# bruno-maruszczak/lap-time-optimization

Measured on AMD Instinct MI355X. Metric: MPC solves/sec (N=40, nx=8 [7 + progress s], nu=2), higher is better.
Workload: dtype f64

## Files before the change

lap-time-optimization_amd/csrc/aux_kernels.h:

```cpp
#pragma once
#include "linearise.h"

namespace ltompc {

template <bool PI = false, bool TS = false>
__device__ __forceinline__ void d_init_slot(const Consts& K, const Work& W, const int k, const int b, const int cold) {
  const int N = W.N;
  double x0[8];
#pragma unroll
  for (int i = 0; i < 8; i++) x0[i] = W.x0[(size_t)i * W.Bp + b];
  if (k == 0) {
#pragma unroll
    for (int i = 0; i < 8; i++) PL(W.X, i, 0, N + 1) = x0[i];
  }
  if (cold) {
#pragma unroll
    for (int i = 0; i < 8; i++) {
      PL(W.X, i, k + 1, N + 1) = x0[i], PL(W.C, i, k, N) = x0[i];
      PL(W.L1, i, k, N) = 0.0, PL(W.L2, i, k, N) = 0.0;
    }
    PL(W.U, 0, k, N) = 0.0, PL(W.U, 1, k, N) = 0.0;
  }
  const int prev = W.si[(size_t)SI_PREV * W.Bp + b];
  const bool resto_ok = K.o.resto_rho > 0.0 && !(K.o.soft_rho > 0.0);
// ... 52 lines not shown
  int b = tid % W.Bp, k = tid / W.Bp;
  if (k >= W.N || b >= W.B) return;
  d_init_slot(K, W, k, b, cold);
}
__global__ void k_init_pi(const Consts* __restrict__ Kp, const WorkPI* __restrict__ Wp, int cold) {
  const Consts& K = *Kp;
  const Work& W = *Wp;
  int tid = blockIdx.x * blockDim.x + threadIdx.x;
  int b = tid % W.Bp, k = tid / W.Bp;
  if (k >= W.N || b >= W.B) return;
  d_init_slot<true>(K, W, k, b, cold);
}
__global__ void k_init_ts(const Consts* __restrict__ Kp, const WorkTS* __restrict__ Wp, int cold) {
  const Consts& K = *Kp;
  const Work& W = *Wp;
  int tid = blockIdx.x * blockDim.x + threadIdx.x;
  int b = tid % W.Bp, k = tid / W.Bp;
  if (k >= W.N || b >= W.B) return;
  d_init_slot<true, true>(K, W, k, b, cold);
}

__global__ void k_shift(Work W, int pass) {
  int tid = blockIdx.x * blockDim.x + threadIdx.x;
  int b = tid % W.Bp, k = tid / W.Bp;
  const int N = W.N;
  if (k > N || b >= W.B) return;
  if (pass == 0) {
    const int kx = k + 1 <= N ? k + 1 : N, ks = k + 1 <= N - 1 ? k + 1 : N - 1;
#pragma unroll
    for (int i = 0; i < 8; i++) PL(W.dX, i, k, N + 1) = PL(W.X, i, kx, N + 1);
    if (k < N) {
#pragma unroll
      for (int i = 0; i < 8; i++) {
        PL(W.dC, i, k, N) = PL(W.C, i, ks, N);
        PL(W.nL1, i, k, N) = PL(W.L1, i, ks, N), PL(W.nL2, i, k, N) = PL(W.L2, i, ks, N);
      }
      PL(W.dU, 0, k, N) = PL(W.U, 0, ks, N), PL(W.dU, 1, k, N) = PL(W.U, 1, ks, N);
    }
  } else {
#pragma unroll
    for (int i = 0; i < 8; i++) PL(W.X, i, k, N + 1) = PL(W.dX, i, k, N + 1);
    if (k < N) {
#pragma unroll
      for (int i = 0; i < 8; i++) {
        PL(W.C, i, k, N) = PL(W.dC, i, k, N);
        PL(W.L1, i, k, N) = PL(W.nL1, i, k, N), PL(W.L2, i, k, N) = PL(W.nL2, i, k, N);
      }
      PL(W.U, 0, k, N) = PL(W.dU, 0, k, N), PL(W.U, 1, k, N) = PL(W.dU, 1, k, N);
    }
  }
}


__global__ void k_act_identity(int* act, int* nact, int B) {
  int b = blockIdx.x * blockDim.x + threadIdx.x;
  if (b < B) act[b] = b;
  if (b == 0) nact[0] = B;
}
__global__ void __launch_bounds__(1024) k_compact(const int* __restrict__ src, const int* __restrict__ nsrc_p,
                                                   const int* __restrict__ done, int* __restrict__ dst, int* __restrict__ ndst) {
  __shared__ int cnt[1024];
  const int t = threadIdx.x, nsrc = nsrc_p[0];
  const int chunk = (nsrc + 1023) / 1024, lo = t * chunk, hi = min(nsrc, lo + chunk);
  int c = 0;
  for (int j = lo; j < hi; j++) c += done[src[j]] ? 0 : 1;
  cnt[t] = c;
  __syncthreads();
  for (int off = 1; off < 1024; off <<= 1) {
    int v = t >= off ? cnt[t - off] : 0;
    __syncthreads();
    cnt[t] += v;
    __syncthreads();
  }
  int pos = cnt[t] - c;
  for (int j = lo; j < hi; j++) {
    int b = src[j];
    if (!done[b]) dst[pos++] = b;
  }
  if (t == 1023) ndst[0] = cnt[1023];
}

__global__ void __launch_bounds__(1024) k_pack_perm(const int* __restrict__ nslots_p, const int* __restrict__ done, int* __restrict__ perm,
                                                     int* __restrict__ act, int* __restrict__ nact) {
  __shared__ int cnt[1024];
  const int t = threadIdx.x, n = nslots_p[0];
  const int chunk = (n + 1023) / 1024, lo = min(n, t * chunk), hi = min(n, lo + chunk);
  int c = 0;
  for (int j = lo; j < hi; j++) c += done[j] ? 0 : 1;
  cnt[t] = c;
  __syncthreads();
  for (int off = 1; off < 1024; off <<= 1) {
    int v = t >= off ? cnt[t - off] : 0;
    __syncthreads();
    cnt[t] += v;
    __syncthreads();
  }
  const int n_act = cnt[1023];
  int pa = cnt[t] - c, pd = n_act + lo - pa;
  for (int j = lo; j < hi; j++) {
    if (!done[j]) act[pa] = pa, perm[pa++] = j;
    else perm[pd++] = j;
  }
  if (t == 0) nact[0] = n_act;
}
__global__ void k_pack_inverse(const int* __restrict__ orig, int* __restrict__ inv, int B) {
  int j = blockIdx.x * blockDim.x + threadIdx.x;
// ... 247 lines not shown
```

lap-time-optimization_amd/csrc/linesearch.h:

```cpp
#pragma once
#include "layout.h"

namespace ltompc {

template <class BP, bool PIN, bool ELL, bool PI = false, bool TS = false>
__device__ __forceinline__ void d_linesearch(const Consts& K, const Work& W, const int k, const int b, const int l_begin,
                                             const int l_end) {
  const int N = W.N;
  const double hdt = K.o.t_step;
  if (W.si[(size_t)SI_DONE * W.Bp + b] || !W.si[(size_t)SI_STEP * W.Bp + b]) return;
  const double eps = W.st[(size_t)ST_EPS * W.Bp + b], rho = W.st[(size_t)ST_RHO * W.Bp + b];
  double a_pri = 1.0;
  for (int kk = 0; kk < N; kk += 20) {
    double v20[20];
#pragma unroll
    for (int q = 0; q < 20; q++) v20[q] = PL(W.SP, SP_apri, kk + q < N ? kk + q : N - 1, N);
#pragma unroll
    for (int q = 0; q < 20; q++) a_pri = fmin(a_pri, v20[q]);
  }
  double xk[8], xp[8], c[8], u[2], v[2], dxk[8], dxp[8], dc[8], du[2], dv[2];
#pragma unroll
  for (int i = 0; i < 8; i++) {
    xk[i] = k == 0 ? W.x0[(size_t)i * W.Bp + b] : PL(W.X, i, k, N + 1);
    dxk[i] = PL(W.dX, i, k, N + 1);
// ... 428 lines not shown
    u[0] = PL(W.U, 0, k, N), u[1] = PL(W.U, 1, k, N), du[0] = PL(W.dU, 0, k, N), du[1] = PL(W.dU, 1, k, N);
#pragma unroll
    for (int i = 0; i < 8; i++) {
      PL(W.X, i, k + 1, N + 1) = x[i] + alpha * dx[i];
      PL(W.C, i, k, N) = c[i] + alpha * dc[i];
      PL(W.L1, i, k, N) = l1[i] + alpha * (n1[i] - l1[i]);
      PL(W.L2, i, k, N) = l2[i] + alpha * (n2[i] - l2[i]);
    }
    PL(W.U, 0, k, N) = u[0] + alpha * du[0], PL(W.U, 1, k, N) = u[1] + alpha * du[1];
  }
  const int ni = K.bd.ni, nel = K.bd.nel, nact = (k + 1 <= N - 1) ? ni : ni - 3 - nel;
  for (int m0 = 0; m0 < nact; m0 += 8) {
    double t[8], dt[8], nu[8], dn[8];
#pragma unroll
    for (int q = 0; q < 8; q++) {
      const int m = m0 + q < nact ? m0 + q : nact - 1;
      t[q] = PL(W.T, m, k, N), dt[q] = PL(W.dT, m, k, N), nu[q] = PL(W.NU, m, k, N), dn[q] = PL(W.dNU, m, k, N);
    }
#pragma unroll
    for (int q = 0; q < 8; q++)
      if (m0 + q < nact) {
        const double tn = t[q] + alpha * dt[q];
        const double nn = nu[q] + a_dua * dn[q];
        const double lo = mu / (1e10 * tn), hi = 1e10 * mu / tn;
        PL(W.T, m0 + q, k, N) = tn, PL(W.NU, m0 + q, k, N) = nn < lo ? lo : (nn > hi ? hi : nn);
      }
  }
  if (W.st[(size_t)ST_RHO * W.Bp + b] > 0.0 && nact == ni) {
    double e[3], de[3];
#pragma unroll
    for (int q = 0; q < 3; q++) e[q] = PL(W.T, ni + q, k, N), de[q] = PL(W.dT, ni + q, k, N);
#pragma unroll
    for (int q = 0; q < 3; q++) PL(W.T, ni + q, k, N) = e[q] + alpha * de[q];
  }
  if (nel && nact == ni) {
    double e[2], de[2];
#pragma unroll
    for (int q = 0; q < 2; q++) e[q] = PL(W.T, ni + 3 + q, k, N), de[q] = PL(W.dT, ni + 3 + q, k, N);
#pragma unroll
    for (int q = 0; q < 2; q++) PL(W.T, ni + 3 + q, k, N) = e[q] + alpha * de[q];
  }
}

__global__ void __launch_bounds__(64) k_update(const Consts* __restrict__ Kp, const Work* __restrict__ Wp, Launch la) {
  const Consts& K = *Kp;
  const Work& W = *Wp;
  int tid = blockIdx.x * blockDim.x + threadIdx.x;
  if (tid == 0) W.ls_count[1] = W.ls_count[0], W.ls_count[0] = 0;
  int j = tid % la.n_pad, k = tid / la.n_pad;
  if (k >= W.N || j >= la.nact[0]) return;
  d_update(K, W, k, la.act[j]);
}


template <class BP, bool ELL>
__global__ void __launch_bounds__(320) k_step1(const Consts* __restrict__ Kp, const Work* __restrict__ Wp, Launch la) {
  const Consts& K = *Kp;
  const Work& W = *Wp;
  if ((int)blockIdx.x >= la.nact[0]) return;
  const int b = la.act[blockIdx.x];
  const int N = W.N, tid = threadIdx.x;
  const int* si = W.si;
  if (si[(size_t)SI_DONE * W.Bp + b] || !si[(size_t)SI_STEP * W.Bp + b]) return;
  const bool rprof = W.DBG != nullptr && blockIdx.x == 0 && tid == 0;
  long long rt0 = rprof ? clock64() : 0;
#define STOCK(q) if (rprof) { const long long t1 = clock64(); W.DBG[q] += (double)(t1 - rt0); rt0 = t1; }
  for (int idx = tid; idx < N * K.o.n_linesearch; idx += 320) d_linesearch<BP, false, ELL>(K, W, idx % N, b, 1 + idx / N, 1 + idx / N);
  STOCK(8);
  __syncthreads();
  STOCK(9);
  if (tid < 64 && (tid & 7) == 0) d_pick(K, W, b, tid >> 3, 1, false);
  __syncthreads();
  STOCK(10);
  for (int kk = tid; kk < N; kk += 320) d_update(K, W, kk, b);
  STOCK(11);
  if (rprof) W.DBG[12] += 1.0;
#undef STOCK
}
template <class BP>
__global__ void __launch_bounds__(320) k_step1_pi(const Consts* __restrict__ Kp, const WorkPI* __restrict__ Wp, Launch la) {
  const Consts& K = *Kp;
  const Work& W = *Wp;
  if ((int)blockIdx.x >= la.nact[0]) return;
  const int b = la.act[blockIdx.x];
  const int N = W.N, tid = threadIdx.x;
  const int* si = W.si;
  if (si[(size_t)SI_DONE * W.Bp + b] || !si[(size_t)SI_STEP * W.Bp + b]) return;
  const bool rprof = W.DBG != nullptr && blockIdx.x == 0 && tid == 0;
  long long rt0 = rprof ? clock64() : 0;
#define STOCK(q) if (rprof) { const long long t1 = clock64(); W.DBG[q] += (double)(t1 - rt0); rt0 = t1; }
  for (int idx = tid; idx < N * K.o.n_linesearch; idx += 320) d_linesearch<BP, false, false, true>(K, W, idx % N, b, 1 + idx / N, 1 + idx / N);
  STOCK(8);
  __syncthreads();
  STOCK(9);
  if (tid < 64 && (tid & 7) == 0) d_pick<true>(K, W, b, tid >> 3, 1, false);
  __syncthreads();
  STOCK(10);
  for (int kk = tid; kk < N; kk += 320) d_update(K, W, kk, b);
  STOCK(11);
  if (rprof) W.DBG[12] += 1.0;
#undef STOCK
}
template <class BP>
__global__ void __launch_bounds__(320) k_step1_ts(const Consts* __restrict__ Kp, const WorkTS* __restrict__ Wp, Launch la) {
  const Consts& K = *Kp;
  const Work& W = *Wp;
  if ((int)blockIdx.x >= la.nact[0]) return;
  const int b = la.act[blockIdx.x];
  const int N = W.N, tid = threadIdx.x;
  const int* si = W.si;
  if (si[(size_t)SI_DONE * W.Bp + b] || !si[(size_t)SI_STEP * W.Bp + b]) return;
  const bool rprof = W.DBG != nullptr && blockIdx.x == 0 && tid == 0;
  long long rt0 = rprof ? clock64() : 0;
#define STOCK(q) if (rprof) { const long long t1 = clock64(); W.DBG[q] += (double)(t1 - rt0); rt0 = t1; }
  for (int idx = tid; idx < N * K.o.n_linesearch; idx += 320) d_linesearch<BP, false, false, true, true>(K, W, idx % N, b, 1 + idx / N, 1 + idx / N);
  STOCK(8);
  __syncthreads();
  STOCK(9);
  if (tid < 64 && (tid & 7) == 0) d_pick<true, true>(K, W, b, tid >> 3, 1, false);
  __syncthreads();
  STOCK(10);
  for (int kk = tid; kk < N; kk += 320) d_update(K, W, kk, b);
  STOCK(11);
  if (rprof) W.DBG[12] += 1.0;
#undef STOCK
}



}
```

lap-time-optimization_amd/csrc/ltompc.hip:

```cpp
#include <hip/hip_runtime.h>

#include <algorithm>
#include <cmath>
#include <cstdio>
#include <cstdlib>
#include <cstring>
#include <string>
#include <type_traits>
#include <vector>

#include "kernels.h"

using namespace ltompc;

namespace {

thread_local std::string g_err;

int fail(const std::string& msg) {
  g_err = msg;
  return -1;
}
#define HIPCHECK(expr)                                                                         \
  do {                                                                                         \
    hipError_t e_ = (expr);                                                                    \
    if (e_ != hipSuccess) return fail(std::string(#expr) + ": " + hipGetErrorString(e_));      \
  } while (0)

constexpr int NKERN = 8;

}

enum class Sens { no_solve, solved, du0, traj };
enum class Psens { none, du0, traj };
struct DerivState {
  Sens sens = Sens::no_solve;
  Psens psens = Psens::none;
  bool fact = false;
  bool pv_valid = false;
  bool kept_uprev = false;
  bool loop_fresh = false;
  int loop_mode = 0;

  void discard() { sens = Sens::no_solve, psens = Psens::none, fact = pv_valid = kept_uprev = false; }
  void solved(const bool kept_u) { sens = Sens::solved, kept_uprev = kept_u, loop_fresh = loop_fresh || kept_u; }
  void moved() { fact = pv_valid = false; }
  void ticked() { loop_fresh = false; }

  Work Ws{}, *d_Ws = nullptr;
  WorkPI Wspi{}, *d_Wspi = nullptr;
  int *d_sens_inertia = nullptr, *d_sens_ok = nullptr;
  double *d_sens_du0 = nullptr, *d_sens_margin = nullptr, *d_sens_dX = nullptr, *d_sens_dU = nullptr;
  double *d_psens_uprev = nullptr, *d_psens_pv = nullptr, *d_psens_kf = nullptr, *d_psens_du0 = nullptr, *d_psens_dX = nullptr,
         *d_psens_dU = nullptr;
  double *d_adj_aj = nullptr, *d_adj_gp = nullptr, *d_adj_gth = nullptr, *d_adj_gX = nullptr, *d_adj_gU = nullptr;
  double *d_psn_planes = nullptr, *d_psn_rm = nullptr, *d_loop_Sx = nullptr, *d_loop_Du = nullptr;
  double *d_jvp_jv = nullptr, *d_jvp_dp = nullptr, *d_jvp_dth = nullptr, *d_jvp_tX = nullptr, *d_jvp_tU = nullptr;
  int *d_loop_ok = nullptr, *d_loop_ticks = nullptr;
  double *d_tab_tj = nullptr, *d_tab_sg = nullptr, *d_tab_gt = nullptr;
  WorkTS Wsts{}, *d_Wsts = nullptr;
  double* d_tab_gs = nullptr;
  int tab_gs_cap = 0;
};

struct ltompc_record_s;

struct ltompc_solver {
  Consts K;
  Work W;
  int device = 0, N = 0, B = 0, Bp = 0, n_table = 0, max_iter = 0;
  hipStream_t own_stream = nullptr, stream = nullptr;
  std::vector<void*> allocs;
  double* d_tables = nullptr;
  double* d_x0_rm = nullptr;
  double* d_u0_rm = nullptr;
  double* d_io = nullptr;
  int* h_active = nullptr;
  int *d_act[2] = {nullptr, nullptr}, *d_nact[2] = {nullptr, nullptr};
  int last_compactions = 0;
  int *d_perm = nullptr, *d_orig = nullptr;
  int ls_width_env = 0;
  int pack_num = 6;
  bool packed = false;
  bool packing = true;
  std::vector<int> history;
  bool cold_next = true;
  int *d_cold = nullptr, *d_inv = nullptr, *d_ws_int = nullptr;
  double* d_ws_stage = nullptr;
  bool cold_pending = false;
  bool uprev_set = false;
  bool after_rollout = false;
  int poll_every = 4;
  int profiling = 0;
  bool compaction = true;
  bool serial_riccati = false;
  std::vector<hipEvent_t> ev, ev_pool;
  size_t ev_pool_used = 0;
  std::vector<int> ev_kind, ev_width, ev_iter;
  std::vector<int> log_kind, log_width, log_iter;
  std::vector<double> log_ms;
  int cur_width = 0;
  int cur_iter = 0;
  int* d_counts = nullptr;
  int solver_counts[8] = {};
  static constexpr int ROLL_RING = 16, ROLL_PLANTS = 4;
  int* d_roll = nullptr;
  int* d_plist = nullptr;
  hipStream_t plant_streams[ROLL_PLANTS] = {};
  int n_plant_streams = 2;
  hipEvent_t ev_fin[ROLL_RING] = {}, ev_done[ROLL_RING] = {};
  long long roll_iterations = 0, roll_launches = 0;
  double ms_by_kernel[NKERN] = {};
  int launches_by_kernel[NKERN] = {};
  Consts* d_K = nullptr;
  Work* d_W = nullptr;
  bool bounds_ref = false;
  bool ref_eval = false, ref_expand = false, ref_ls = false, ref_step1 = false;
  bool eval8 = true;
  int step1_width = 512;
  int sweeps_width = 16;
  int ric1q_width = 16;
  int ric1_width = 512;
  int last_launches = 0, last_iterations = 0;
  DerivState dv;
  double *d_th_pend = nullptr, *d_th_solve = nullptr;
  bool pi_pend = false, pi_solve = false;
  bool pi_narrow = true;
  WorkPI Wpi{};
  WorkPI* d_Wpi = nullptr;
  int n_sets = 0, ts_cap = 0;
// ... 455 lines not shown
    if (s1) h->step1_width = atoi(s1);
    const char* t = getenv("LTOMPC_RIC1");
    if (t) h->ric1_width = atoi(t);
    const char* npl = getenv("LTOMPC_PLANT_STREAMS");
    if (npl) h->n_plant_streams = std::min((int)ltompc_solver::ROLL_PLANTS, std::max(1, std::atoi(npl)));
    const char* sw = getenv("LTOMPC_SWEEPS_W");
    if (sw) h->sweeps_width = atoi(sw);
    const char* rq = getenv("LTOMPC_RIC1Q");
    if (rq) h->ric1q_width = atoi(rq);
    if (std::max(ric1_lds_bytes(n_horizon), ric1q_lds_bytes(n_horizon)) > 150 * 1024) h->ric1_width = 0;
    else if (hipFuncSetAttribute(reinterpret_cast<const void*>(k_riccati1), hipFuncAttributeMaxDynamicSharedMemorySize, 150 * 1024) != hipSuccess ||
             hipFuncSetAttribute(reinterpret_cast<const void*>(k_riccati1q), hipFuncAttributeMaxDynamicSharedMemorySize, 150 * 1024) != hipSuccess) {
      (void)hipGetLastError();
      h->ric1_width = 0;
    }
    if (h->ric1_width > 0 &&
        (hipFuncSetAttribute(reinterpret_cast<const void*>(k_riccati1_pi), hipFuncAttributeMaxDynamicSharedMemorySize, 150 * 1024) != hipSuccess ||
         hipFuncSetAttribute(reinterpret_cast<const void*>(k_riccati1q_pi), hipFuncAttributeMaxDynamicSharedMemorySize, 150 * 1024) != hipSuccess)) {
      (void)hipGetLastError();
      h->pi_narrow = false;
    }
  }
  const size_t N = h->N, Bp = h->Bp;
  const int ni = h->K.bd.ni;
  Work& W = h->W;
  W.N = h->N, W.B = h->B, W.Bp = h->Bp;
  int rc = 0;
  rc |= h->dalloc(&h->d_tables, (size_t)LTOMPC_TABLE_ROWS * n_table);
  rc |= h->dalloc(&W.X, 8 * (N + 1) * Bp, true), rc |= h->dalloc(&W.C, 8 * N * Bp, true), rc |= h->dalloc(&W.U, 2 * N * Bp, true);
  rc |= h->dalloc(&W.L1, 8 * N * Bp, true), rc |= h->dalloc(&W.L2, 8 * N * Bp, true);
  const size_t nel = h->K.bd.nel;
  rc |= h->dalloc(&W.T, (ni + NNL + nel) * N * Bp, true), rc |= h->dalloc(&W.NU, ni * N * Bp, true);
  rc |= h->dalloc(&W.dX, 8 * (N + 1) * Bp, true), rc |= h->dalloc(&W.dC, 8 * N * Bp, true), rc |= h->dalloc(&W.dU, 2 * N * Bp, true);
  rc |= h->dalloc(&W.nL1, 8 * N * Bp, true), rc |= h->dalloc(&W.nL2, 8 * N * Bp, true);
  rc |= h->dalloc(&W.dT, (ni + NNL + nel) * N * Bp, true), rc |= h->dalloc(&W.dNU, ni * N * Bp, true);
  rc |= h->dalloc(&W.QP, (size_t)QP_NF * (N + 1) * Bp, true), rc |= h->dalloc(&W.RC, (size_t)RC_NF * (N + 1) * Bp, true);
  rc |= h->dalloc(&W.RS, (size_t)RS_NF * N * Bp, true), rc |= h->dalloc(&W.SP, (size_t)SP_NF * N * Bp, true);
  rc |= h->dalloc(&W.LS, (size_t)3 * (options->n_linesearch + 1) * N * Bp, true);
  rc |= h->dalloc(&W.x0, 8 * Bp), rc |= h->dalloc(&W.uprev, 2 * Bp), rc |= h->dalloc(&h->dv.d_psens_uprev, 2 * Bp);
  rc |= h->dalloc(&W.st, (size_t)ST_NF * Bp), rc |= h->dalloc(&W.filt, (size_t)2 * FILTER_MAX * Bp);
  rc |= h->dalloc(&W.si, (size_t)SI_NF * Bp), rc |= h->dalloc(&W.active, (size_t)h->max_iter + 2);
  rc |= h->dalloc(&h->d_act[0], Bp), rc |= h->dalloc(&h->d_act[1], Bp), rc |= h->dalloc(&h->d_nact[0], 4), rc |= h->dalloc(&h->d_nact[1], 4);
  rc |= h->dalloc(&W.ls_list, Bp), rc |= h->dalloc(&W.ls_count, 4);
  rc |= h->dalloc(&h->d_perm, Bp), rc |= h->dalloc(&h->d_orig, Bp);
  rc |= h->dalloc(&W.BK, 18 * N * Bp, true);
  rc |= h->dalloc(&h->d_counts, 32), rc |= h->dalloc(&h->d_roll, 2 * ltompc_solver::ROLL_RING);
  rc |= h->dalloc(&h->d_plist, (size_t)ltompc_solver::ROLL_RING * h->Bp);
  if (getenv("LTOMPC_DBG")) rc |= h->dalloc(&W.DBG, 8 * N * Bp);
  rc |= h->dalloc(&h->d_x0_rm, 8 * Bp), rc |= h->dalloc(&h->d_u0_rm, 2 * Bp), rc |= h->dalloc(&h->d_io, 32 * Bp);
  if (rc) {
    ltompc_destroy(h);
    return -1;
  }
  if (hipHostMalloc((void**)&h->h_active, sizeof(int) * 4) != hipSuccess) {
    ltompc_destroy(h);
    return fail("hipHostMalloc failed");
  }
  W.orig = (gptr<const int>)h->d_orig;
  hipLaunchKernelGGL(k_act_identity, dim3((h->B + 63) / 64), dim3(64), 0, h->stream, h->d_orig, h->d_perm, h->B);
  if (hipMemcpyAsync(h->d_tables, tables, sizeof(double) * LTOMPC_TABLE_ROWS * n_table, hipMemcpyHostToDevice, h->stream) != hipSuccess ||
      hipStreamSynchronize(h->stream) != hipSuccess) {
    ltompc_destroy(h);
    return fail("table upload failed");
  }
  Tables& T = h->K.T;
  T.n = n_table;
  using tp = gptr<const double>;
  T.s_kappa = (tp)h->d_tables, T.kappa = (tp)(h->d_tables + n_table), T.s_arc = (tp)(h->d_tables + 2 * (size_t)n_table);
  T.n_left = (tp)(h->d_tables + 3 * (size_t)n_table), T.n_right = (tp)(h->d_tables + 4 * (size_t)n_table), T.v_ref = (tp)(h->d_tables + 5 * (size_t)n_table);
  T.g0_kappa = tables[0], T.inv_kappa = (double)(n_table - 1) / (tables[n_table - 1] - tables[0]);
  T.period = options->periodic_tables ? tables[n_table - 1] - tables[0] : 0.0;
  T.g0_arc = tables[2 * (size_t)n_table], T.inv_arc = (double)(n_table - 1) / (tables[3 * (size_t)n_table - 1] - tables[2 * (size_t)n_table]);
  if (h->dalloc(&h->d_K, 1) || h->dalloc(&h->d_W, 1) ||
      hipMemcpyAsync(h->d_K, &h->K, sizeof(Consts), hipMemcpyHostToDevice, h->stream) != hipSuccess ||
      hipMemcpyAsync(h->d_W, &h->W, sizeof(Work), hipMemcpyHostToDevice, h->stream) != hipSuccess ||
      hipStreamSynchronize(h->stream) != hipSuccess) {
    ltompc_destroy(h);
    return fail("ltompc_create: upload of the constants failed");
  }
  *out = h;
  return 0;
}

int ltompc_destroy(ltompc_handle h) {
  if (!h) return 0;
  (void)hipSetDevice(h->device);
  if (h->stream) (void)hipStreamSynchronize(h->stream);
  for (void* p : h->allocs) (void)hipFree(p);
  for (ltompc_record_s* r : h->recs) delete r;
  for (hipEvent_t e : h->ev_pool) (void)hipEventDestroy(e);
  if (h->h_active) (void)hipHostFree(h->h_active);
  if (h->own_stream) (void)hipStreamDestroy(h->own_stream);
  for (auto& ps : h->plant_streams)
    if (ps) (void)hipStreamDestroy(ps);
  for (int i = 0; i < ltompc_solver::ROLL_RING; i++) {
    if (h->ev_fin[i]) (void)hipEventDestroy(h->ev_fin[i]);
    if (h->ev_done[i]) (void)hipEventDestroy(h->ev_done[i]);
  }
  delete h;
  return 0;
}

int ltompc_set_stream(ltompc_handle h, void* hip_stream) {
  if (!h) return fail("null handle");
  h->stream = hip_stream ? static_cast<hipStream_t>(hip_stream) : h->own_stream;
  return 0;
}
// ... 200 lines not shown
  const bool ell = h->K.bd.nel > 0;
  Launcher L{h};
  h->dv.discard();
  if (commit_theta(h)) return -1;
  const bool per_inst = h->cold_pending;
  if (per_inst) hipLaunchKernelGGL(k_load_x0_m, dim3((B + 63) / 64), dim3(64), 0, h->stream, h->W, x0_dev, h->K.o.resto_sticky, (const int*)h->d_cold);
  else
  hipLaunchKernelGGL(k_load_x0, dim3((B + 63) / 64), dim3(64), 0, h->stream, h->W, x0_dev, (const int*)(h->packed ? h->d_orig : nullptr),
                     h->K.o.resto_sticky, h->cold_next ? 0 : 1);
  if (h->cold_next && !h->uprev_set) hipLaunchKernelGGL(k_zero_uprev, dim3((B + 63) / 64), dim3(64), 0, h->stream, h->W);
  h->uprev_set = false;
  if (!h->cold_next && h->K.o.warm_shift) {
    hipLaunchKernelGGL(k_shift, dim3(((N + 1) * Bp + 63) / 64), dim3(64), 0, h->stream, h->W, 0);
    hipLaunchKernelGGL(k_shift, dim3(((N + 1) * Bp + 63) / 64), dim3(64), 0, h->stream, h->W, 1);
  }
  if (per_inst) {
    if (h->ts_solve) hipLaunchKernelGGL(k_init_m_ts, dim3((N * Bp + 63) / 64), dim3(64), 0, h->stream, h->d_K, h->d_Wts, (const int*)h->d_cold);
    else if (h->pi_solve) hipLaunchKernelGGL(k_init_m_pi, dim3((N * Bp + 63) / 64), dim3(64), 0, h->stream, h->d_K, h->d_Wpi, (const int*)h->d_cold);
    else hipLaunchKernelGGL(k_init_m, dim3((N * Bp + 63) / 64), dim3(64), 0, h->stream, h->d_K, h->d_W, (const int*)h->d_cold);
    HIPCHECK(hipMemsetAsync(h->d_cold, 0, sizeof(int) * Bp, h->stream));
    h->cold_pending = false;
  } else if (h->ts_solve) hipLaunchKernelGGL(k_init_ts, dim3((N * Bp + 63) / 64), dim3(64), 0, h->stream, h->d_K, h->d_Wts, h->cold_next ? 1 : 0);
  else if (h->pi_solve) hipLaunchKernelGGL(k_init_pi, dim3((N * Bp + 63) / 64), dim3(64), 0, h->stream, h->d_K, h->d_Wpi, h->cold_next ? 1 : 0);
  else hipLaunchKernelGGL(k_init, dim3((N * Bp + 63) / 64), dim3(64), 0, h->stream, h->d_K, h->d_W, h->cold_next ? 1 : 0);
  HIPCHECK(hipMemsetAsync(h->W.active, 0, sizeof(int) * ((size_t)h->max_iter + 2), h->stream));
  HIPCHECK(hipMemsetAsync(h->W.ls_count, 0, 2 * sizeof(int), h->stream));
  h->cold_next = false, h->after_rollout = false;
  int cur = 0, n_launch = B;
  hipLaunchKernelGGL(k_act_identity, dim3((B + 63) / 64), dim3(64), 0, h->stream, h->d_act[0], h->d_nact[0], B);
  Launch la{};
  auto set_launch = [&](int n) {
    n_launch = n;
    h->cur_width = n;
    la.act = (gptr<const int>)h->d_act[cur], la.nact = (gptr<const int>)h->d_nact[cur], la.n_pad = (n + 63) / 64 * 64;
  };
  set_launch(B);
  h->last_compactions = 0;
  h->history.clear();
  int it = 0;
  bool force_eval_next = false;
  int ls_width = h->ls_width_env ? h->ls_width_env : 512;
  for (;; it++) {
    const int np = la.n_pad;
    h->cur_iter = it;
    la.force_eval = force_eval_next ? 1 : 0;
    force_eval_next = false;
    {
      const int rc = launch_iteration(h, L, la, it, n_launch, ls_width, ell, it >= h->max_iter);
      if (rc < 0) return -1;
    }
    if (it >= h->max_iter) break;
    if ((it + 1) % h->poll_every == 0) {
      if (L.close()) return -1;
      HIPCHECK(hipMemcpyAsync(h->h_active, h->W.active + it, sizeof(int), hipMemcpyDeviceToHost, h->stream));
      HIPCHECK(hipMemcpyAsync(h->h_active + 1, h->W.ls_count + 1, sizeof(int), hipMemcpyDeviceToHost, h->stream));
      HIPCHECK(hipStreamSynchronize(h->stream));
      const int n_active = h->h_active[0];
      if (h->ls_width_env == 0) {
        const int last = h->h_active[1];
        ls_width = std::min(std::max(64, (last + last / 2 + 63) / 64 * 64), 2048);
      }
      h->history.push_back(it), h->history.push_back(n_active), h->history.push_back(n_launch);
      if (n_active == 0) break;
      if (h->compaction && n_active <= (h->pack_num * n_launch) / 8) {
        if (h->packing && n_launch > 512) {
          if (!h->packed) hipLaunchKernelGGL(k_act_identity, dim3((B + 63) / 64), dim3(64), 0, h->stream, h->d_orig, h->d_perm, B);
          h->packed = true;
          hipLaunchKernelGGL(k_pack_perm, dim3(1), dim3(1024), 0, h->stream, h->d_nact[cur], h->W.si + (size_t)SI_DONE * Bp, h->d_perm,
                             h->d_act[cur ^ 1], h->d_nact[cur ^ 1]);
          const int nthreads = (N + 1) * n_launch;
          for (int pass = 0; pass < 2; pass++)
            hipLaunchKernelGGL(k_pack, dim3((nthreads + 255) / 256), dim3(256), 0, h->stream, h->W, h->d_perm, h->d_nact[cur], n_launch,
                               h->d_orig, h->K.bd.ni, h->K.bd.nel, pass);
          force_eval_next = true;
        } else {
          hipLaunchKernelGGL(k_compact, dim3(1), dim3(1024), 0, h->stream, h->d_act[cur], h->d_nact[cur],
                             h->W.si + (size_t)SI_DONE * Bp, h->d_act[cur ^ 1], h->d_nact[cur ^ 1]);
        }
        cur ^= 1;
        set_launch(n_active);
        h->last_compactions++;
      }
    }
  }
  if (L.close()) return -1;
  hipLaunchKernelGGL(k_psens_keep_uprev, dim3((B + 63) / 64), dim3(64), 0, h->stream, h->W, h->dv.d_psens_uprev, (const int*)(h->packed ? h->d_orig : nullptr));
  hipLaunchKernelGGL(k_store_u0, dim3((B + 63) / 64), dim3(64), 0, h->stream, h->W, u0_dev, (const int*)(h->packed ? h->d_orig : nullptr));
  HIPCHECK(hipGetLastError());
  h->last_launches = L.launches + 3;
  h->last_iterations = it + 1;
  h->dv.solved(true);
  if (h->profiling) {
    HIPCHECK(hipStreamSynchronize(h->stream));
    if (collect_profile(h)) return -1;
  }
  return 0;
}

int ltompc_synchronize(ltompc_handle h) {
  if (!h) return fail("null handle");
  HIPCHECK(hipSetDevice(h->device));
  HIPCHECK(hipStreamSynchronize(h->stream));
  return 0;
}

int ltompc_get_stats(ltompc_handle h, int* status, int* iters, double* kkt_error, double* objective, double* mu) {
  std::vector<int> si;
  std::vector<double> st;
// ... 89 lines not shown
  const int ring = h->max_iter + 2;
  long long it = 0;
  bool first = true;
  int rc = 0;
#define ROLLCHECK(expr)                                                                          \
  {                                                                                              \
    hipError_t e_ = (expr);                                                                      \
    if (e_ != hipSuccess) { rc = fail(std::string(#expr) + ": " + hipGetErrorString(e_)); break; } \
  }
  for (;; it++) {
    const int np = la.n_pad, slot = (int)(it % RING);
    int* const d_cnt = h->d_roll + 2 * slot;
    int* const d_list = h->d_plist + (size_t)slot * Bp;
    if (done_pending[slot]) ROLLCHECK(hipStreamWaitEvent(h->stream, h->ev_done[slot], 0));
    ROLLCHECK(hipMemsetAsync(d_cnt, 0, 2 * sizeof(int), h->stream));
    if (first && h->cold_pending) {
      hipLaunchKernelGGL(k_roll_mark_m, dim3((B + 63) / 64), dim3(64), 0, h->stream, h->W, (const double*)x_dev, h->K.o.resto_sticky, (const int*)h->d_cold);
      if (h->ts_solve) hipLaunchKernelGGL(k_roll_init_m_ts, dim3((N * np + 63) / 64), dim3(64), 0, h->stream, h->d_K, h->d_Wts, la, (const int*)h->d_cold);
      else if (h->pi_solve) hipLaunchKernelGGL(k_roll_init_m_pi, dim3((N * np + 63) / 64), dim3(64), 0, h->stream, h->d_K, h->d_Wpi, la, (const int*)h->d_cold);
      else hipLaunchKernelGGL(k_roll_init_m, dim3((N * np + 63) / 64), dim3(64), 0, h->stream, h->d_K, h->d_W, la, (const int*)h->d_cold);
      ROLLCHECK(hipMemsetAsync(h->d_cold, 0, sizeof(int) * Bp, h->stream));
      h->cold_pending = false;
    } else {
    hipLaunchKernelGGL(k_roll_mark, dim3((B + 63) / 64), dim3(64), 0, h->stream, h->W, (const double*)x_dev, h->K.o.resto_sticky,
                       (first && h->cold_next) ? 1 : 0);
    if (h->ts_solve)
      hipLaunchKernelGGL(k_roll_init_ts, dim3((N * np + 63) / 64), dim3(64), 0, h->stream, h->d_K, h->d_Wts, la, (first && h->cold_next) ? 1 : 0);
    else if (h->pi_solve)
      hipLaunchKernelGGL(k_roll_init_pi, dim3((N * np + 63) / 64), dim3(64), 0, h->stream, h->d_K, h->d_Wpi, la, (first && h->cold_next) ? 1 : 0);
    else hipLaunchKernelGGL(k_roll_init, dim3((N * np + 63) / 64), dim3(64), 0, h->stream, h->d_K, h->d_W, la, (first && h->cold_next) ? 1 : 0);
    }
    la.force_eval = 0;
    if (launch_iteration(h, L, la, -1, n_launch, ls_width, ell, false) < 0) { rc = -1; break; }
    hipLaunchKernelGGL(k_roll_finish, dim3((np + 63) / 64), dim3(64), 0, h->stream, h->W, la, u_log_dev, status_log_dev, iters_log_dev, n_ticks,
                       d_cnt, d_list);
    {
      hipStream_t ps = h->plant_streams[it % h->n_plant_streams];
      ROLLCHECK(hipEventRecord(h->ev_fin[slot], h->stream));
      ROLLCHECK(hipStreamWaitEvent(ps, h->ev_fin[slot], 0));
      if (h->ts_solve)
        hipLaunchKernelGGL(k_roll_plant_ts, dim3((n_launch + 63) / 64), dim3(64), 0, ps, h->K, h->Wts, x_dev, h->K.o.t_step, n_sub, (const int*)(d_cnt + 1),
                           (const int*)d_list);
      else if (h->pi_solve)
        hipLaunchKernelGGL(k_roll_plant_pi, dim3((n_launch + 63) / 64), dim3(64), 0, ps, h->K, h->Wpi, x_dev, h->K.o.t_step, n_sub, (const int*)(d_cnt + 1),
                           (const int*)d_list);
      else
      hipLaunchKernelGGL(k_roll_plant, dim3((n_launch + 63) / 64), dim3(64), 0, ps, h->K, h->W, x_dev, h->K.o.t_step, n_sub, (const int*)(d_cnt + 1),
                         (const int*)d_list);
      ROLLCHECK(hipEventRecord(h->ev_done[slot], ps));
      done_pending[slot] = true;
    }
    first = false;
    if ((it + 1) % h->poll_every == 0) {
      ROLLCHECK(hipMemcpyAsync(h->h_active, d_cnt, sizeof(int), hipMemcpyDeviceToHost, h->stream));
      ROLLCHECK(hipMemcpyAsync(h->h_active + 1, h->W.ls_count + 1, sizeof(int), hipMemcpyDeviceToHost, h->stream));
      ROLLCHECK(hipStreamSynchronize(h->stream));
      const int n_left = h->h_active[0];
      h->history.push_back((int)it), h->history.push_back(n_left), h->history.push_back(n_launch);
      if (h->ls_width_env == 0) {
        const int last = h->h_active[1];
        ls_width = std::min(std::max(64, (last + last / 2 + 63) / 64 * 64), 2048);
      }
      if (n_left == 0) break;
      if (it >= it_cap) { rc = fail("ltompc_rollout: iteration cap reached (internal error)"); break; }
      if (h->compaction && n_left <= (h->pack_num * n_launch) / 8) {
        hipLaunchKernelGGL(k_compact, dim3(1), dim3(1024), 0, h->stream, h->d_act[cur], h->d_nact[cur], h->W.si + (size_t)SI_FINAL * Bp,
                           h->d_act[cur ^ 1], h->d_nact[cur ^ 1]);
        cur ^= 1;
        set_launch(n_left);
      }
    }
  }
#undef ROLLCHECK
  for (int i = 0; i < h->n_plant_streams; i++)
    if (hipStreamSynchronize(h->plant_streams[i]) != hipSuccess && rc == 0) rc = fail("ltompc_rollout: plant stream failed");
  if (hipStreamSynchronize(h->stream) != hipSuccess && rc == 0) rc = fail("ltompc_rollout: solver stream failed");
  if (hipGetLastError() != hipSuccess && rc == 0) rc = fail("ltompc_rollout: a kernel launch failed");
  h->profiling = prof;
  h->cold_next = false;
  h->roll_iterations = it + 1, h->roll_launches = L.launches;
  h->last_iterations = 0;
  h->after_rollout = true;
  if (rc == 0) h->dv.solved(false);
  return rc;
}

int ltompc_get_prediction_dev(ltompc_handle h, double* X_dev, double* U_dev) {
  if (!h) return fail("null handle");
  if (!X_dev && !U_dev) return 0;
  HIPCHECK(hipSetDevice(h->device));
  const size_t nthreads = (size_t)(h->N + 1) * h->Bp;
  hipLaunchKernelGGL(k_prediction_dev, dim3((unsigned)((nthreads + 255) / 256)), dim3(256), 0, h->stream, h->W, X_dev, U_dev);
  HIPCHECK(hipGetLastError());
  return 0;
}

int ltompc_set_instance_params(ltompc_handle h, const double* theta) {
  static const char* names[LTOMPC_NTHETA] = {"mass", "inertia_z", "B_f", "C_f", "D_f", "B_r", "C_r", "D_r", "C_m", "Cr_0", "Cr_2",
                                             "q_n", "q_mu", "q_B", "r_du[0]", "r_du[1]"};
  if (!h) return fail("null handle");
  if (!theta) {
    h->pi_pend = false;
    return 0;
  }
  const char* who = "ltompc_set_instance_params";
  for (int b = 0; b < h->B; b++)
    for (int j = 0; j < LTOMPC_NTHETA; j++) {
      const double v = theta[(size_t)b * LTOMPC_NTHETA + j];
// ... 308 lines not shown
```

Baseline: 169,300.

## Prefetch update operands during pick phase and poll via zero-copy kernel

In the step1 kernels, threads 64-319 are idle while the first 64 threads run d_pick. They now preload the primal, dual and slack update operands into registers during that phase. After the barrier they apply the step with the chosen alpha, and only fall back to the old loop for the shift case and for rows beyond the preloaded range. Separately, the two device-to-host memcpys used for host polling are replaced by a tiny kernel that writes both values into mapped pinned host memory. The aim is to hide update load latency behind the pick and to cut per-poll copy overhead, at the cost of higher register pressure and more complex indexing.

```diff
diff --git a/lap-time-optimization_amd/csrc/aux_kernels.h b/lap-time-optimization_amd/csrc/aux_kernels.h
--- a/lap-time-optimization_amd/csrc/aux_kernels.h
+++ b/lap-time-optimization_amd/csrc/aux_kernels.h
@@ -128,6 +128,10 @@
 }
 
 
+__global__ void __launch_bounds__(64) k_poll(const int* __restrict__ n_active, const int* __restrict__ ls_last, int* __restrict__ out) {
+  if (blockIdx.x == 0 && threadIdx.x == 0) out[0] = n_active[0], out[1] = ls_last[0];
+}
+
 __global__ void k_act_identity(int* act, int* nact, int B) {
   int b = blockIdx.x * blockDim.x + threadIdx.x;
   if (b < B) act[b] = b;
diff --git a/lap-time-optimization_amd/csrc/linesearch.h b/lap-time-optimization_amd/csrc/linesearch.h
--- a/lap-time-optimization_amd/csrc/linesearch.h
+++ b/lap-time-optimization_amd/csrc/linesearch.h
@@ -504,6 +504,114 @@
   d_update(K, W, k, la.act[j]);
 }
 
+constexpr int UPD_ROUNDS = 2;
+constexpr int UPD_QUADS = 3;
+struct UpdRow {
+  double a[5], d[5], e, de;
+  double t[UPD_QUADS], dt[UPD_QUADS], nu[UPD_QUADS], dn[UPD_QUADS];
+};
+struct UpdRegs {
+  UpdRow row[UPD_ROUNDS];
+};
+
+__device__ __forceinline__ void upd_load_pairs(const Consts& K, const Work& W, const int k, const int r, const int b, UpdRow& v) {
+  const int N = W.N, ni = K.bd.ni, nel = K.bd.nel;
+  const int ru = r < 2 ? r : 1, re = ni + (r < 3 + nel ? r : 0);
+  v.a[0] = PL(W.X, r, k + 1, N + 1), v.d[0] = PL(W.dX, r, k + 1, N + 1), v.a[1] = PL(W.C, r, k, N), v.d[1] = PL(W.dC, r, k, N);
+  v.a[2] = PL(W.L1, r, k, N), v.d[2] = PL(W.nL1, r, k, N), v.a[3] = PL(W.L2, r, k, N), v.d[3] = PL(W.nL2, r, k, N);
+  v.a[4] = PL(W.U, ru, k, N), v.d[4] = PL(W.dU, ru, k, N);
+  v.e = PL(W.T, re, k, N), v.de = PL(W.dT, re, k, N);
+}
+__device__ __forceinline__ void upd_load_quads(const Consts& K, const Work& W, const int k, const int r, const int b, const int m0, UpdRow& v) {
+  const int N = W.N, ni = K.bd.ni, nel = K.bd.nel, nact = (k + 1 <= N - 1) ? ni : ni - 3 - nel;
+  const int last = nact > 0 ? nact - 1 : 0;
+#pragma unroll
+  for (int q = 0; q < UPD_QUADS; q++) {
+    const int m = m0 + r + 8 * q < nact ? m0 + r + 8 * q : last;
+    v.t[q] = PL(W.T, m, k, N), v.dt[q] = PL(W.dT, m, k, N), v.nu[q] = PL(W.NU, m, k, N), v.dn[q] = PL(W.dNU, m, k, N);
+  }
+}
+__device__ __forceinline__ void upd_store_pairs(const Consts& K, const Work& W, const int k, const int r, const int b, const double alpha,
+                                                const double rho, const UpdRow& v) {
+  const int N = W.N, ni = K.bd.ni, nel = K.bd.nel;
+  PL(W.X, r, k + 1, N + 1) = v.a[0] + alpha * v.d[0];
+  PL(W.C, r, k, N) = v.a[1] + alpha * v.d[1];
+  PL(W.L1, r, k, N) = v.a[2] + alpha * (v.d[2] - v.a[2]);
+  PL(W.L2, r, k, N) = v.a[3] + alpha * (v.d[3] - v.a[3]);
+  if (r < 2) PL(W.U, r, k, N) = v.a[4] + alpha * v.d[4];
+  if (k + 1 <= N - 1 && (r < 3 ? rho > 0.0 : r < 3 + nel)) PL(W.T, ni + r, k, N) = v.e + alpha * v.de;
+}
+__device__ __forceinline__ void upd_store_quads(const Consts& K, const Work& W, const int k, const int r, const int b, const int m0,
+                                                const double alpha, const double a_dua, const double mu, const UpdRow& v) {
+  const int N = W.N, ni = K.bd.ni, nel = K.bd.nel, nact = (k + 1 <= N - 1) ? ni : ni - 3 - nel;
+#pragma unroll
+  for (int q = 0; q < UPD_QUADS; q++)
+    if (m0 + r + 8 * q < nact) {
+      const double tn = v.t[q] + alpha * v.dt[q];
+      const double nn = v.nu[q] + a_dua * v.dn[q];
+      const double lo = mu / (1e10 * tn), hi = 1e10 * mu / tn;
+      PL(W.T, m0 + r + 8 * q, k, N) = tn, PL(W.NU, m0 + r + 8 * q, k, N) = nn < lo ? lo : (nn > hi ? hi : nn);
+    }
+}
+
+__device__ __forceinline__ void d_update_fetch(const Consts& K, const Work& W, const int tid, const int b, UpdRegs& R) {
+  const int N = W.N, w = tid - 64;
+#pragma unroll
+  for (int j = 0; j < UPD_ROUNDS; j++) {
+    const int k = 32 * j + (w >> 3);
+    if (k < N) upd_load_pairs(K, W, k, w & 7, b, R.row[j]), upd_load_quads(K, W, k, w & 7, b, 0, R.row[j]);
+  }
+#if defined(__HIP_DEVICE_COMPILE__)
+#pragma unroll
+  for (int j = 0; j < UPD_ROUNDS; j++) {
+    UpdRow& v = R.row[j];
+    asm volatile("" : "+v"(v.a[0]), "+v"(v.d[0]), "+v"(v.a[1]), "+v"(v.d[1]), "+v"(v.a[2]), "+v"(v.d[2]), "+v"(v.a[3]), "+v"(v.d[3]),
+                 "+v"(v.a[4]), "+v"(v.d[4]), "+v"(v.e), "+v"(v.de));
+    asm volatile("" : "+v"(v.t[0]), "+v"(v.dt[0]), "+v"(v.nu[0]), "+v"(v.dn[0]), "+v"(v.t[1]), "+v"(v.dt[1]), "+v"(v.nu[1]), "+v"(v.dn[1]),
+                 "+v"(v.t[2]), "+v"(v.dt[2]), "+v"(v.nu[2]), "+v"(v.dn[2]));
+  }
+#endif
+}
+
+__device__ __forceinline__ void d_update_store(const Consts& K, const Work& W, const int tid, const int b, const UpdRegs& R) {
+  const int N = W.N;
+  int shift = W.si[(size_t)SI_SHIFT * W.Bp + b], done = W.si[(size_t)SI_DONE * W.Bp + b], step = W.si[(size_t)SI_STEP * W.Bp + b];
+  double alpha = W.st[(size_t)ST_ALPHA * W.Bp + b], a_dua = W.st[(size_t)ST_ADUA * W.Bp + b];
+  double mu = W.st[(size_t)ST_MU * W.Bp + b], rho = W.st[(size_t)ST_RHO * W.Bp + b];
+#if defined(__HIP_DEVICE_COMPILE__)
+  asm volatile("" : "+v"(shift), "+v"(done), "+v"(step), "+v"(alpha), "+v"(a_dua), "+v"(mu), "+v"(rho));
+#endif
+  if (shift && !done) {
+    for (int kk = tid; kk < N; kk += 320) {
+#if defined(__clang__)
+      __builtin_assume(W.si[(size_t)SI_SHIFT * W.Bp + b] && !W.si[(size_t)SI_DONE * W.Bp + b]);
+#endif
+      d_update(K, W, kk, b);
+    }
+    return;
+  }
+  if (!step || done || tid < 64) return;
+  const int w = tid - 64, r = w & 7;
+#pragma unroll
+  for (int j = 0; j < UPD_ROUNDS; j++) {
+    const int k = 32 * j + (w >> 3);
+    if (k < N) upd_store_pairs(K, W, k, r, b, alpha, rho, R.row[j]), upd_store_quads(K, W, k, r, b, 0, alpha, a_dua, mu, R.row[j]);
+  }
+  const int ni = K.bd.ni;
+  if (N <= UPD_ROUNDS * 32 && ni <= UPD_QUADS * 8) return;
+  for (int k = w >> 3; k < N; k += 32) {
+    UpdRow v;
+    if (k >= UPD_ROUNDS * 32) {
+      upd_load_pairs(K, W, k, r, b, v), upd_load_quads(K, W, k, r, b, 0, v);
+      upd_store_pairs(K, W, k, r, b, alpha, rho, v), upd_store_quads(K, W, k, r, b, 0, alpha, a_dua, mu, v);
+    }
+    for (int m0 = UPD_QUADS * 8; m0 < ni; m0 += UPD_QUADS * 8) {
+      upd_load_quads(K, W, k, r, b, m0, v);
+      upd_store_quads(K, W, k, r, b, m0, alpha, a_dua, mu, v);
+    }
+  }
+}
+
 
 template <class BP, bool ELL>
 __global__ void __launch_bounds__(320) k_step1(const Consts* __restrict__ Kp, const Work* __restrict__ Wp, Launch la) {
@@ -521,10 +629,13 @@
   STOCK(8);
   __syncthreads();
   STOCK(9);
-  if (tid < 64 && (tid & 7) == 0) d_pick(K, W, b, tid >> 3, 1, false);
+  UpdRegs upd;
+  if (tid < 64) {
+    if ((tid & 7) == 0) d_pick(K, W, b, tid >> 3, 1, false);
+  } else d_update_fetch(K, W, tid, b, upd);
   __syncthreads();
   STOCK(10);
-  for (int kk = tid; kk < N; kk += 320) d_update(K, W, kk, b);
+  d_update_store(K, W, tid, b, upd);
   STOCK(11);
   if (rprof) W.DBG[12] += 1.0;
 #undef STOCK
@@ -545,10 +656,13 @@
   STOCK(8);
   __syncthreads();
   STOCK(9);
-  if (tid < 64 && (tid & 7) == 0) d_pick<true>(K, W, b, tid >> 3, 1, false);
+  UpdRegs upd;
+  if (tid < 64) {
+    if ((tid & 7) == 0) d_pick<true>(K, W, b, tid >> 3, 1, false);
+  } else d_update_fetch(K, W, tid, b, upd);
   __syncthreads();
   STOCK(10);
-  for (int kk = tid; kk < N; kk += 320) d_update(K, W, kk, b);
+  d_update_store(K, W, tid, b, upd);
   STOCK(11);
   if (rprof) W.DBG[12] += 1.0;
 #undef STOCK
@@ -569,10 +683,13 @@
   STOCK(8);
   __syncthreads();
   STOCK(9);
-  if (tid < 64 && (tid & 7) == 0) d_pick<true, true>(K, W, b, tid >> 3, 1, false);
+  UpdRegs upd;
+  if (tid < 64) {
+    if ((tid & 7) == 0) d_pick<true, true>(K, W, b, tid >> 3, 1, false);
+  } else d_update_fetch(K, W, tid, b, upd);
   __syncthreads();
   STOCK(10);
-  for (int kk = tid; kk < N; kk += 320) d_update(K, W, kk, b);
+  d_update_store(K, W, tid, b, upd);
   STOCK(11);
   if (rprof) W.DBG[12] += 1.0;
 #undef STOCK
diff --git a/lap-time-optimization_amd/csrc/ltompc.hip b/lap-time-optimization_amd/csrc/ltompc.hip
--- a/lap-time-optimization_amd/csrc/ltompc.hip
+++ b/lap-time-optimization_amd/csrc/ltompc.hip
@@ -76,6 +76,7 @@
   double* d_u0_rm = nullptr;
   double* d_io = nullptr;
   int* h_active = nullptr;
+  int* h_active_dev = nullptr;
   int *d_act[2] = {nullptr, nullptr}, *d_nact[2] = {nullptr, nullptr};
   int last_compactions = 0;
   int *d_perm = nullptr, *d_orig = nullptr;
@@ -637,7 +638,8 @@
     ltompc_destroy(h);
     return -1;
   }
-  if (hipHostMalloc((void**)&h->h_active, sizeof(int) * 4) != hipSuccess) {
+  if (hipHostMalloc((void**)&h->h_active, sizeof(int) * 4) != hipSuccess ||
+      hipHostGetDevicePointer((void**)&h->h_active_dev, h->h_active, 0) != hipSuccess) {
     ltompc_destroy(h);
     return fail("hipHostMalloc failed");
   }
@@ -944,8 +946,7 @@
     if (it >= h->max_iter) break;
     if ((it + 1) % h->poll_every == 0) {
       if (L.close()) return -1;
-      HIPCHECK(hipMemcpyAsync(h->h_active, h->W.active + it, sizeof(int), hipMemcpyDeviceToHost, h->stream));
-      HIPCHECK(hipMemcpyAsync(h->h_active + 1, h->W.ls_count + 1, sizeof(int), hipMemcpyDeviceToHost, h->stream));
+      hipLaunchKernelGGL(k_poll, dim3(1), dim3(64), 0, h->stream, (const int*)(h->W.active + it), (const int*)(h->W.ls_count + 1), h->h_active_dev);
       HIPCHECK(hipStreamSynchronize(h->stream));
       const int n_active = h->h_active[0];
       if (h->ls_width_env == 0) {
@@ -1141,8 +1142,7 @@
     }
     first = false;
     if ((it + 1) % h->poll_every == 0) {
-      ROLLCHECK(hipMemcpyAsync(h->h_active, d_cnt, sizeof(int), hipMemcpyDeviceToHost, h->stream));
-      ROLLCHECK(hipMemcpyAsync(h->h_active + 1, h->W.ls_count + 1, sizeof(int), hipMemcpyDeviceToHost, h->stream));
+      hipLaunchKernelGGL(k_poll, dim3(1), dim3(64), 0, h->stream, (const int*)d_cnt, (const int*)(h->W.ls_count + 1), h->h_active_dev);
       ROLLCHECK(hipStreamSynchronize(h->stream));
       const int n_left = h->h_active[0];
       h->history.push_back((int)it), h->history.push_back(n_left), h->history.push_back(n_launch);
```

Measured after the change: 171,500 (median of 6 runs). 1.01x the previous value.
